# SHI-Labs/Self-Similarity-Grouping

Hardware: AMD Instinct MI355X
Metric: images/s embed + s/iter for NxN rerank+DBSCAN, N=16k, 1/2/4/8 GPU (higher is better)
Workload: dtype f32 (embed: split-half operands hi+lo on fp16 MFMA, fp32 accumulate, 6e-8 max error vs the fp32 reference features) / exact int64 via int8 MFMA digits + f64 + f16 (distance, re-rank: half semantics, bit-exact)

## Files before the change

### self-similarity-grouping_amd/csrc/bottleneck.hip

```cpp
#include "ssg_common.h"
#include <cstdlib>

#ifndef SSG_BN_NT_STORE
#define SSG_BN_NT_STORE 1
#endif
#ifndef SSG_BN_NT_RES
#define SSG_BN_NT_RES 1
#endif

namespace ssg {
namespace bneck {

typedef float v16f __attribute__((ext_vector_type(16)));
typedef unsigned int v4u __attribute__((ext_vector_type(4)));
typedef _Float16 v8h __attribute__((ext_vector_type(8)));
typedef float v4f __attribute__((ext_vector_type(4)));

struct Params {
  const float* x; float* out;
  const float* w1; const float* b1; const float* cs1;
  const float* w2; const float* b2; const float* cs2;
  const float* w3; const float* b3; const float* cs3;
  int B, H;
  int* overflow;
  unsigned long long* prof = nullptr;
};
#ifdef SSG_BN_PROF
#define SSG_BN_STAMP(I_) { if (p.prof && threadIdx.x == 0) p.prof[(size_t)blockIdx.x * 8 + (I_)] = __builtin_readcyclecounter(); }
#else
#define SSG_BN_STAMP(I_)
#endif

constexpr int cmax(int a, int b) { return a > b ? a : b; }

template <int C, int MID, int IW, int TH, int CIN = C, int NW = 4>
struct Cfg {
  static constexpr int HROWS = TH + 2, NPIX1 = HROWS * IW, NPIX = TH * IW;
  static constexpr int NTHR = NW * 64, RPP = NTHR / 4;
#ifndef SSG_BN_K1T
#define SSG_BN_K1T 32
#endif
#ifndef SSG_BN_K1T4
#define SSG_BN_K1T4 32
#endif
  static constexpr int K1T = NW == 8 ? SSG_BN_K1T : SSG_BN_K1T4, KS1 = K1T / 16, CPR1 = 4 * KS1, RPP1 = NTHR / CPR1;
  static constexpr int XROWS = (NPIX1 + RPP1 - 1) / RPP1 * RPP1;
  static constexpr int P1 = 80;
  static constexpr int P1T = K1T * 4 + 16;
  static constexpr int KT2 = NW == 8 ? 2 : 1;
  static constexpr int P2 = KT2 * 128 + 16;
  static constexpr int PY = MID * 4 + 16;
  static constexpr int BUF1 = (XROWS + MID) * P1T;
  static constexpr int ZERO_OFF = NPIX1 * PY;
  static constexpr int W2_OFF = (ZERO_OFF + PY + 255) / 256 * 256, BUF2 = MID * P2;
  static constexpr int W3_OFF = (NPIX * PY + 255) / 256 * 256, BUF3 = C * P1;
  static constexpr int LDS = cmax(cmax(2 * BUF1, W2_OFF + 2 * BUF2), W3_OFF + 2 * BUF3);
  static constexpr int DS = CIN != C;
#ifdef SSG_BN_ABL_NK1
  static constexpr int NK1 = SSG_BN_ABL_NK1;
#else
  static constexpr int NK1 = CIN / K1T;
#endif
  static constexpr int NK2 = (MID / 32) * 9 / KT2, NK3 = (MID + (DS ? CIN : 0)) / 16;
  static constexpr int PD1MAX = K1T == 64 ? 2 : (K1T == 32 ? 4 : 8);
  static constexpr int PD1 = NK1 < PD1MAX ? NK1 : PD1MAX, PD2 = KT2 == 1 ? 6 : 3;
  static_assert(((MID / 32) * 9) % KT2 == 0 && NK2 % PD2 == 0, "phase-2 stages and ring");
  static_assert((NW == 4 || NW == 8) && NPIX == 128 && NPIX1 % 32 == 0 && MID % RPP == 0 && MID % RPP1 == 0 && C % RPP == 0 && MID % (NW * 8) == 0, "128 output pixels, whole staging passes");
  static constexpr bool ZERO_EARLY = 2 * BUF1 <= ZERO_OFF;
  static_assert(LDS <= (NW == 4 ? 80 : 160) * 1024, "4 waves: two workgroups per CU; 8 waves: one");
  static_assert(NW == 4 || NW * 32 * 36 * 4 <= 2 * BUF3, "8 waves: the epilogue patches take over the W3 stages");
};

__device__ __forceinline__ unsigned pack2(_Float16 a, _Float16 b) {
  return (unsigned)__builtin_bit_cast(unsigned short, a) | ((unsigned)__builtin_bit_cast(unsigned short, b) << 16);
}
__device__ __forceinline__ void encode4(const float4 v, uint2& hi, uint2& lo) {
  const _Float16 h0 = (_Float16)v.x, h1 = (_Float16)v.y, h2 = (_Float16)v.z, h3 = (_Float16)v.w;
  hi = make_uint2(pack2(h0, h1), pack2(h2, h3));
  lo = make_uint2(pack2((_Float16)(v.x - (float)h0), (_Float16)(v.y - (float)h1)), pack2((_Float16)(v.z - (float)h2), (_Float16)(v.w - (float)h3)));
}
__device__ __forceinline__ unsigned hi_nonfinite_bits(const uint2 hi) {
  return ((hi.x & 0x7c007c00u) + 0x04000400u) | ((hi.y & 0x7c007c00u) + 0x04000400u);
}
__device__ __forceinline__ float hlo(unsigned u) { return (float)__builtin_bit_cast(_Float16, (unsigned short)(u & 0xffffu)); }
__device__ __forceinline__ float hhi(unsigned u) { return (float)__builtin_bit_cast(_Float16, (unsigned short)(u >> 16)); }
__device__ __forceinline__ float4 decode4(const uint2 hi, const uint2 lo) {
  return make_float4(hlo(hi.x) + hlo(lo.x), hhi(hi.x) + hhi(lo.x), hlo(hi.y) + hlo(lo.y), hhi(hi.y) + hhi(lo.y));
}
__device__ __forceinline__ float4 relu4(float4 v) {
  return make_float4(v.x > 0.f ? v.x : 0.f, v.y > 0.f ? v.y : 0.f, v.z > 0.f ? v.z : 0.f, v.w > 0.f ? v.w : 0.f);
}

__device__ __forceinline__ void bn_dma16(const __amdgpu_buffer_rsrc_t r, unsigned lds_addr, unsigned voff, int soff) {
  __builtin_amdgcn_raw_ptr_buffer_load_lds(r, (__attribute__((address_space(3))) void*)(uintptr_t)lds_addr, 16, voff, soff, 0, 0);
}

template <int C, int MID, int IW, int TH, int CIN, int NW>
__global__ __launch_bounds__(NW * 64, NW == 4 ? 2 : 1) void bottleneck_kernel(Params p) {
  using K = Cfg<C, MID, IW, TH, CIN, NW>;
  constexpr bool DS = K::DS;
  extern __shared__ __attribute__((aligned(16))) unsigned char smem[];
  const int tid = (int)threadIdx.x, lane = tid & 63, wave = tid >> 6, l32 = lane & 31, h = lane >> 5;
  const int tiles_img = p.H / TH, ntiles = p.B * tiles_img;
  int T;
  {
    const int b = (int)blockIdx.x, q = ntiles / 8, r = ntiles % 8, x = b % 8, s = b / 8;
    T = (x < r ? x * (q + 1) : r * (q + 1) + (x - r) * q) + s;
  }
  const int img = T / tiles_img, ty0 = (T - img * tiles_img) * TH;
  SSG_BN_STAMP(0)
  if (K::ZERO_EARLY && tid < K::PY / 16) *reinterpret_cast<uint4*>(smem + K::ZERO_OFF + tid * 16) = make_uint4(0u, 0u, 0u, 0u);

  constexpr int RPP = K::RPP, RPP1 = K::RPP1, AU = K::XROWS / RPP1, WU = MID / RPP1;
  const int ck = tid & 3, r0 = tid >> 2;
  const int ck1 = tid % K::CPR1, r1 = tid / K::CPR1;
  const float* ximg = p.x + (int64_t)img * p.H * IW * CIN;
  const __amdgpu_buffer_rsrc_t xrsrc = __builtin_amdgcn_make_buffer_rsrc(const_cast<float*>(ximg), 0, (unsigned)(p.H * IW * CIN * 4), 0x00020000);
  constexpr int MT1 = K::NPIX1 / 32, NT1 = MID / 32;
  constexpr int WC1 = NT1 < NW / 2 ? NT1 : NW / 2, WR1 = NW / WC1, MTW1 = (MT1 + WR1 - 1) / WR1, NTW1 = NT1 / WC1;
  static_assert(NT1 % WC1 == 0 && (WR1 * MTW1) * 32 <= K::XROWS, "phase-1 tiles divide over the waves");
  const int i1b = (wave / WC1) * MTW1, j1b = (wave % WC1) * NTW1;
  v16f acc1[MTW1][NTW1];
#pragma unroll
  for (int i = 0; i < MTW1; i++)
#pragma unroll
    for (int j = 0; j < NTW1; j++)
#pragma unroll
      for (int r = 0; r < 16; r++) acc1[i][j][r] = 0.f;
  float4 cs1r[NTW1][4], b1r[NTW1][4];
#pragma unroll
  for (int j = 0; j < NTW1; j++)
#pragma unroll
    for (int q = 0; q < 4; q++) {
      cs1r[j][q] = *reinterpret_cast<const float4*>(p.cs1 + (j1b + j) * 32 + 8 * q + 4 * h); b1r[j][q] = *reinterpret_cast<const float4*>(p.b1 + (j1b + j) * 32 + 8 * q + 4 * h);
    }
#ifndef SSG_BN_P1DMA
#define SSG_BN_P1DMA 1
#endif
  if constexpr (NW == 8 && K::K1T == 32 && SSG_BN_P1DMA) {
    constexpr int NS = 4, XR = K::NPIX1, SROWS = XR + MID, STG = SROWS * 128, NBLK = SROWS / 8, TDMA = (NBLK + NW - 1) / NW;
    static_assert(K::NK1 % NS == 0 && NS * STG <= K::LDS && SROWS % 8 == 0 && XR % 8 == 0 && MTW1 == 3 && NTW1 == 1, "phase-1 DMA stages");
    const int wv = __builtin_amdgcn_readfirstlane(wave);
    const __amdgpu_buffer_rsrc_t wrsrc = __builtin_amdgcn_make_buffer_rsrc(const_cast<float*>(p.w1), 0, (unsigned)(MID * CIN * 4), 0x00020000);
    unsigned go[TDMA];
    int gblk[TDMA];
#pragma unroll
    for (int u = 0; u < TDMA; u++) {
      int blk = wv + NW * u;
      if (blk >= NBLK) blk = wv;
      gblk[u] = blk;
      const int r = blk * 8 + (lane >> 3), lc = (lane & 7) ^ ((r >> 1) & 7);
      if (blk < XR / 8) {
        const int pix = (ty0 - 1) * IW + r;
        go[u] = (pix >= 0 && pix < p.H * IW) ? (unsigned)((pix * CIN + lc * 4) * 4) : 0x80000000u;
      } else {
        go[u] = (unsigned)(((r - XR) * CIN + lc * 4) * 4);
      }
    }
#define SSG_BN_DMA1(T_, ST_)                                                                                         \
    { _Pragma("unroll") for (int u = 0; u < TDMA; u++)                                                               \
        bn_dma16(gblk[u] < XR / 8 ? xrsrc : wrsrc, (unsigned)(uintptr_t)(smem + (ST_) * STG + gblk[u] * 1024), go[u], (T_) * 128); }
    const int i1s = __builtin_amdgcn_readfirstlane(i1b);
    int xo[MTW1], xs[MTW1];
#pragma unroll
    for (int i = 0; i < MTW1; i++) { const int r = (i1s + i) * 32 + l32; xo[i] = r * 128; xs[i] = (r >> 1) & 7; }
    const int wr_ = XR + j1b * 32 + l32, wo = wr_ * 128, ws = (wr_ >> 1) & 7;
    v8h fxh[2][2][MTW1], fxl[2][2][MTW1], fwh[2][2], fwl[2][2];
#define SSG_BN_READS1(ST_, S_)                                                                                       \
    { const unsigned char* sb_ = smem + (ST_) * STG;                                                                 \
      _Pragma("unroll") for (int ks = 0; ks < 2; ks++) {                                                             \
        _Pragma("unroll") for (int i = 0; i < MTW1; i++) {                                        \
          fxh[S_][ks][i] = *reinterpret_cast<const v8h*>(sb_ + xo[i] + (((4 * ks + 2 * h) ^ xs[i]) * 16));           \
          fxl[S_][ks][i] = *reinterpret_cast<const v8h*>(sb_ + xo[i] + (((4 * ks + 2 * h + 1) ^ xs[i]) * 16)); }     \
        fwh[S_][ks] = *reinterpret_cast<const v8h*>(sb_ + wo + (((4 * ks + 2 * h) ^ ws) * 16));                       \
        fwl[S_][ks] = *reinterpret_cast<const v8h*>(sb_ + wo + (((4 * ks + 2 * h + 1) ^ ws) * 16)); } }
#define SSG_BN_MMAK(S_, KS_)                                                                                         \
    { _Pragma("unroll") for (int i = 0; i < MTW1; i++) acc1[i][0] = __builtin_amdgcn_mfma_f32_32x32x16_f16(fwh[S_][KS_], fxl[S_][KS_][i], acc1[i][0], 0, 0, 0); \
      _Pragma("unroll") for (int i = 0; i < MTW1; i++) acc1[i][0] = __builtin_amdgcn_mfma_f32_32x32x16_f16(fwl[S_][KS_], fxh[S_][KS_][i], acc1[i][0], 0, 0, 0); \
      _Pragma("unroll") for (int i = 0; i < MTW1; i++) acc1[i][0] = __builtin_amdgcn_mfma_f32_32x32x16_f16(fwh[S_][KS_], fxh[S_][KS_][i], acc1[i][0], 0, 0, 0); }
#define SSG_BN_STEPD(KT_, ST_, STN_, S_)                                                                             \
    { SSG_BN_MMAK(S_, 0)                                                                                             \
      __builtin_amdgcn_sched_barrier(0);                                                                             \
      asm volatile("s_waitcnt vmcnt(%0) lgkmcnt(0)\n\ts_barrier" ::"n"(TDMA * (NS - 2)) : "memory");                  \
      { const int tn_ = (KT_) + NS < K::NK1 ? (KT_) + NS : K::NK1 - 1;    \
        SSG_BN_DMA1(tn_, ST_) }                                                                                      \
      SSG_BN_READS1(STN_, 1 - (S_))                                                                                  \
      __builtin_amdgcn_sched_barrier(0);                                                                             \
      SSG_BN_MMAK(S_, 1) }
    SSG_BN_DMA1(0, 0) SSG_BN_DMA1(1, 1) SSG_BN_DMA1(2, 2) SSG_BN_DMA1(3, 3)
    asm volatile("s_waitcnt vmcnt(%0)\n\ts_barrier" ::"n"(TDMA * (NS - 1)) : "memory");
    SSG_BN_READS1(0, 0)
#pragma unroll 1
    for (int kt = 0; kt < K::NK1; kt += NS) {
      SSG_BN_STEPD(kt, 0, 1, 0) SSG_BN_STEPD(kt + 1, 1, 2, 1) SSG_BN_STEPD(kt + 2, 2, 3, 0) SSG_BN_STEPD(kt + 3, 3, 0, 1)
    }
    __syncthreads();
#undef SSG_BN_STEPD
#undef SSG_BN_MMAK
#undef SSG_BN_READS1
#undef SSG_BN_DMA1
  } else {
  unsigned aoff[AU];
#pragma unroll
  for (int u = 0; u < AU; u++) {
    const int hp = r1 + RPP1 * u, pix = (ty0 - 1) * IW + hp;
    aoff[u] = (hp < K::NPIX1 && pix >= 0 && pix < p.H * IW) ? (unsigned)((pix * CIN + ck1 * 4) * 4) : 0x80000000u;
  }
  const float* w1p = p.w1 + (int64_t)r1 * CIN + ck1 * 4;
  v4f sa[K::PD1][AU], sw[K::PD1][WU];
#define SSG_BN_LOAD1(T_, S_)                                                                                         \
  {                                                                                                                  \
    _Pragma("unroll") for (int u = 0; u < AU; u++) {                                                                  \
      const v4u raw = __builtin_amdgcn_raw_buffer_load_b128(xrsrc, aoff[u], (T_) * (K::K1T * 4), 0);                  \
      sa[S_][u] = __builtin_bit_cast(v4f, raw);                                                                     \
    }                                                                                                                 \
    _Pragma("unroll") for (int u = 0; u < WU; u++) sw[S_][u] = *reinterpret_cast<const v4f*>(w1p + (int64_t)(RPP1 * u) * CIN + (T_) * K::K1T); \
  }
#define SSG_BN_STORE1(BUF_, S_)                                                                                      \
  {                                                                                                                  \
    unsigned char* sb_ = smem + (BUF_) * K::BUF1;                                                                    \
    _Pragma("unroll") for (int u = 0; u < AU; u++) *reinterpret_cast<v4f*>(sb_ + (r1 + RPP1 * u) * K::P1T + ck1 * 16) = sa[S_][u]; \
    _Pragma("unroll") for (int u = 0; u < WU; u++) *reinterpret_cast<v4f*>(sb_ + (K::XROWS + r1 + RPP1 * u) * K::P1T + ck1 * 16) = sw[S_][u]; \
  }
#define SSG_BN_MMA1(BUF_)                                                                                            \
  {                                                                                                                  \
    const unsigned char* sb_ = smem + (BUF_) * K::BUF1;                                                              \
    _Pragma("unroll") for (int ks = 0; ks < K::KS1; ks++) {                                                          \
    v8h xh_[MTW1], xl_[MTW1], wh_[NTW1], wl_[NTW1];                                                                  \
    _Pragma("unroll") for (int i = 0; i < MTW1; i++) {                                                               \
      const unsigned char* q_ = sb_ + ((i1b + i) * 32 + l32) * K::P1T + ks * 64 + h * 32;                            \
      xh_[i] = *reinterpret_cast<const v8h*>(q_); xl_[i] = *reinterpret_cast<const v8h*>(q_ + 16); }                 \
    _Pragma("unroll") for (int j = 0; j < NTW1; j++) {                                                               \
      const unsigned char* q_ = sb_ + (K::XROWS + (j1b + j) * 32 + l32) * K::P1T + ks * 64 + h * 32;                 \
      wh_[j] = *reinterpret_cast<const v8h*>(q_); wl_[j] = *reinterpret_cast<const v8h*>(q_ + 16); }                 \
    _Pragma("unroll") for (int i = 0; i < MTW1; i++) _Pragma("unroll") for (int j = 0; j < NTW1; j++)                \
      acc1[i][j] = __builtin_amdgcn_mfma_f32_32x32x16_f16(wh_[j], xl_[i], acc1[i][j], 0, 0, 0);                      \
    _Pragma("unroll") for (int i = 0; i < MTW1; i++) _Pragma("unroll") for (int j = 0; j < NTW1; j++)                \
      acc1[i][j] = __builtin_amdgcn_mfma_f32_32x32x16_f16(wl_[j], xh_[i], acc1[i][j], 0, 0, 0);                      \
    _Pragma("unroll") for (int i = 0; i < MTW1; i++) _Pragma("unroll") for (int j = 0; j < NTW1; j++)                \
      acc1[i][j] = __builtin_amdgcn_mfma_f32_32x32x16_f16(wh_[j], xh_[i], acc1[i][j], 0, 0, 0);                      \
    }                                                                                                                \
  }
#define SSG_BN_STEP1(KT_, S_)                                                                                        \
  {                                                                                                                  \
    if ((KT_) + K::PD1 < K::NK1) SSG_BN_LOAD1((KT_) + K::PD1, S_)    \
    SSG_BN_MMA1((S_) & 1)                                                                                            \
    if ((KT_) + 1 < K::NK1) SSG_BN_STORE1(((S_) + 1) & 1, ((S_) + 1) % K::PD1)                                        \
    __syncthreads();                                                                                                 \
  }
  static_assert(K::NK1 % K::PD1 == 0 && K::PD1 <= 8, "phase-1 ring of PD1 register sets");
#define SSG_BN_LOAD1_IF(S_) if constexpr ((S_) < K::PD1) SSG_BN_LOAD1(S_, S_)
  SSG_BN_LOAD1_IF(0) SSG_BN_LOAD1_IF(1) SSG_BN_LOAD1_IF(2) SSG_BN_LOAD1_IF(3) SSG_BN_LOAD1_IF(4) SSG_BN_LOAD1_IF(5) SSG_BN_LOAD1_IF(6) SSG_BN_LOAD1_IF(7)
#undef SSG_BN_LOAD1_IF
  SSG_BN_STORE1(0, 0)
  __syncthreads();
#define SSG_BN_STEP1_IF(KT_, S_) if constexpr ((S_) < K::PD1) SSG_BN_STEP1(KT_, S_)
#pragma unroll
  for (int kt0 = 0; kt0 < K::NK1; kt0 += K::PD1) {
    SSG_BN_STEP1_IF(kt0, 0) SSG_BN_STEP1_IF(kt0 + 1, 1) SSG_BN_STEP1_IF(kt0 + 2, 2) SSG_BN_STEP1_IF(kt0 + 3, 3)
    SSG_BN_STEP1_IF(kt0 + 4, 4) SSG_BN_STEP1_IF(kt0 + 5, 5) SSG_BN_STEP1_IF(kt0 + 6, 6) SSG_BN_STEP1_IF(kt0 + 7, 7)
  }
#undef SSG_BN_STEP1_IF
#undef SSG_BN_STEP1
  }
  SSG_BN_STAMP(1)
#undef SSG_BN_LOAD1
#undef SSG_BN_STORE1
#undef SSG_BN_MMA1

  constexpr int CPR2 = 8 * K::KT2, RP8 = K::NTHR / CPR2, BU = MID / RP8;
  const int ck8 = tid % CPR2, r8 = tid / CPR2;
  const float* w2p = p.w2 + (int64_t)r8 * (9 * MID) + ck8 * 4;
  v4f sb2[K::PD2][BU];
#define SSG_BN_LOAD2(T_, S_)                                                                                         \
  { _Pragma("unroll") for (int u = 0; u < BU; u++) sb2[S_][u] = *reinterpret_cast<const v4f*>(w2p + (int64_t)(RP8 * u) * (9 * MID) + (T_) * (32 * K::KT2)); }
#define SSG_BN_STORE2(BUF_, S_)                                                                                      \
  { unsigned char* sb_ = smem + K::W2_OFF + (BUF_) * K::BUF2;                                                        \
    _Pragma("unroll") for (int u = 0; u < BU; u++) *reinterpret_cast<v4f*>(sb_ + (r8 + RP8 * u) * K::P2 + ck8 * 16) = sb2[S_][u]; }
#define SSG_BN_LOAD2_IF(S_) if constexpr ((S_) < K::PD2) SSG_BN_LOAD2(S_, S_)
  SSG_BN_LOAD2_IF(0) SSG_BN_LOAD2_IF(1) SSG_BN_LOAD2_IF(2) SSG_BN_LOAD2_IF(3) SSG_BN_LOAD2_IF(4) SSG_BN_LOAD2_IF(5)
#undef SSG_BN_LOAD2_IF

  unsigned ovf = 0u;
#pragma unroll
  for (int i = 0; i < MTW1; i++) {
    if (i1b + i >= MT1) continue;
    const int hp0 = (i1b + i) * 32;
    const int irow = ty0 - 1 + (hp0 + l32) / IW;
    const bool inside = irow >= 0 && irow < p.H;
#pragma unroll
    for (int j = 0; j < NTW1; j++)
#pragma unroll
      for (int q = 0; q < 4; q++) {
        const int ch = (j1b + j) * 32 + 8 * q + 4 * h;
        const float4 cs = cs1r[j][q], bi = b1r[j][q];
        float4 v = make_float4(acc1[i][j][4 * q] * cs.x + bi.x, acc1[i][j][4 * q + 1] * cs.y + bi.y, acc1[i][j][4 * q + 2] * cs.z + bi.z,
                               acc1[i][j][4 * q + 3] * cs.w + bi.w);
        v = relu4(v);
        if (!inside) v = make_float4(0.f, 0.f, 0.f, 0.f);
        uint2 hi, lo;
        encode4(v, hi, lo);
        ovf |= hi_nonfinite_bits(hi);
        unsigned char* d = smem + (hp0 + l32) * K::PY + (ch >> 3) * 32 + h * 8;
        *reinterpret_cast<uint2*>(d) = hi; *reinterpret_cast<uint2*>(d + 16) = lo;
      }
  }
  if (!K::ZERO_EARLY && tid < K::PY / 16) *reinterpret_cast<uint4*>(smem + K::ZERO_OFF + tid * 16) = make_uint4(0u, 0u, 0u, 0u);
  SSG_BN_STORE2(0, 0)
  __syncthreads();
  SSG_BN_STAMP(2)

  constexpr int WC2 = NW / 4, NT2 = MID / 32 / WC2;
  const int pt2 = wave / WC2, cb2 = (wave % WC2) * NT2;
  v16f acc2[NT2];
#pragma unroll
  for (int j = 0; j < NT2; j++)
#pragma unroll
    for (int r = 0; r < 16; r++) acc2[j][r] = 0.f;
  const int m2 = pt2 * 32 + l32, ty2 = m2 / IW, tx2 = m2 - ty2 * IW;
  float4 cs2r[NT2][4], b2r[NT2][4];
#pragma unroll
  for (int j = 0; j < NT2; j++)
#pragma unroll
    for (int q = 0; q < 4; q++) {
      cs2r[j][q] = *reinterpret_cast<const float4*>(p.cs2 + (cb2 + j) * 32 + 8 * q + 4 * h); b2r[j][q] = *reinterpret_cast<const float4*>(p.b2 + (cb2 + j) * 32 + 8 * q + 4 * h);
    }
#define SSG_BN_STEP2(KT_, S_, B_)                                                                                     \
  {                                                                                                                  \
    if ((KT_) + K::PD2 < K::NK2) SSG_BN_LOAD2((KT_) + K::PD2, S_)                                                     \
    _Pragma("unroll") for (int sub = 0; sub < K::KT2; sub++) {                                                       \
      const int kt_ = (KT_) * K::KT2 + sub;                                                                          \
      const int chunk = kt_ / 9, tap = kt_ - chunk * 9, r = tap / 3, s = tap - r * 3;                                \
      const int xin = tx2 + s - 1;                                                                                   \
      const int abase = (xin >= 0 && xin < IW) ? ((ty2 + r) * IW + xin) * K::PY : K::ZERO_OFF;                       \
      const unsigned char* wb = smem + K::W2_OFF + (B_) * K::BUF2 + (cb2 * 32 + l32) * K::P2 + sub * 128 + h * 32;     \
      v8h xh_[2], xl_[2], wh_[2][NT2], wl_[2][NT2];                                                                  \
      _Pragma("unroll") for (int ks = 0; ks < 2; ks++) {                                                             \
        const unsigned char* q_ = smem + abase + (chunk * 4 + ks * 2 + h) * 32;                                      \
        xh_[ks] = *reinterpret_cast<const v8h*>(q_); xl_[ks] = *reinterpret_cast<const v8h*>(q_ + 16);               \
        _Pragma("unroll") for (int j = 0; j < NT2; j++) {                                                            \
          wh_[ks][j] = *reinterpret_cast<const v8h*>(wb + j * 32 * K::P2 + ks * 64);                                 \
          wl_[ks][j] = *reinterpret_cast<const v8h*>(wb + j * 32 * K::P2 + ks * 64 + 16); }                          \
      }                                                                                                              \
      _Pragma("unroll") for (int ks = 0; ks < 2; ks++) {                                                             \
        _Pragma("unroll") for (int j = 0; j < NT2; j++) acc2[j] = __builtin_amdgcn_mfma_f32_32x32x16_f16(wh_[ks][j], xl_[ks], acc2[j], 0, 0, 0); \
        _Pragma("unroll") for (int j = 0; j < NT2; j++) acc2[j] = __builtin_amdgcn_mfma_f32_32x32x16_f16(wl_[ks][j], xh_[ks], acc2[j], 0, 0, 0); \
        _Pragma("unroll") for (int j = 0; j < NT2; j++) acc2[j] = __builtin_amdgcn_mfma_f32_32x32x16_f16(wh_[ks][j], xh_[ks], acc2[j], 0, 0, 0); \
      }                                                                                                              \
    }                                                                                                                \
    if ((KT_) + 1 < K::NK2) SSG_BN_STORE2((B_) ^ 1, ((S_) + 1) % K::PD2)                                              \
    __syncthreads();                                                                                                 \
  }
  static_assert(K::NK2 % 6 == 0 && 6 % K::PD2 == 0, "phase-2 ring");
#pragma unroll
  for (int kt0 = 0; kt0 < K::NK2; kt0 += 6) {
    SSG_BN_STEP2(kt0, 0 % K::PD2, 0) SSG_BN_STEP2(kt0 + 1, 1 % K::PD2, 1) SSG_BN_STEP2(kt0 + 2, 2 % K::PD2, 0)
    SSG_BN_STEP2(kt0 + 3, 3 % K::PD2, 1) SSG_BN_STEP2(kt0 + 4, 4 % K::PD2, 0) SSG_BN_STEP2(kt0 + 5, 5 % K::PD2, 1)
  }
#undef SSG_BN_STEP2
  SSG_BN_STAMP(3)
#undef SSG_BN_LOAD2
#undef SSG_BN_STORE2

  constexpr int CU3 = C / RPP;
  constexpr int K3 = MID + (DS ? CIN : 0);
  const float* w3p = p.w3 + (int64_t)r0 * K3 + ck * 4;
  v4f sc3[2][CU3];
#define SSG_BN_LOAD3(T_, S_)                                                                                         \
  { _Pragma("unroll") for (int u = 0; u < CU3; u++) sc3[S_][u] = *reinterpret_cast<const v4f*>(w3p + (int64_t)(RPP * u) * K3 + (T_) * 16); }
#define SSG_BN_STORE3(BUF_, S_)                                                                                      \
  { unsigned char* sb_ = smem + K::W3_OFF + (BUF_) * K::BUF3;                                                        \
    _Pragma("unroll") for (int u = 0; u < CU3; u++) *reinterpret_cast<v4f*>(sb_ + (r0 + RPP * u) * K::P1 + ck * 16) = sc3[S_][u]; }
  SSG_BN_LOAD3(0, 0)
  SSG_BN_LOAD3(1, 1)
  constexpr int WC3 = NW / 4, NT3 = C / 32 / WC3;
  const int pt3 = wave / WC3, cb3 = (wave % WC3) * NT3;
  const int64_t gpix0 = ((int64_t)img * p.H + ty0) * IW + pt3 * 32;
  constexpr int NXK = DS ? CIN / 16 : 1;
  v8h xrh[NXK], xrl[NXK];
  if constexpr (DS) {
    const float* xq = p.x + (gpix0 + l32) * CIN + h * 8;
#pragma unroll
    for (int t = 0; t < NXK; t++) { xrh[t] = *reinterpret_cast<const v8h*>(xq + t * 16); xrl[t] = *reinterpret_cast<const v8h*>(xq + t * 16 + 4); }
  }
  unsigned char* myrows = smem + (pt3 * 32) * K::PY;
#pragma unroll
  for (int j = 0; j < NT2; j++)
#pragma unroll
    for (int q = 0; q < 4; q++) {
      const int ch = (cb2 + j) * 32 + 8 * q + 4 * h;
      const float4 cs = cs2r[j][q], bi = b2r[j][q];
      float4 v = make_float4(acc2[j][4 * q] * cs.x + bi.x, acc2[j][4 * q + 1] * cs.y + bi.y, acc2[j][4 * q + 2] * cs.z + bi.z, acc2[j][4 * q + 3] * cs.w + bi.w);
      v = relu4(v);
      uint2 hi, lo;
      encode4(v, hi, lo);
      ovf |= hi_nonfinite_bits(hi);
      unsigned char* d = smem + (pt2 * 32 + l32) * K::PY + (ch >> 3) * 32 + h * 8;
      *reinterpret_cast<uint2*>(d) = hi; *reinterpret_cast<uint2*>(d + 16) = lo;
    }

  static_assert(K::NK3 % 2 == 0, "phase 3 takes its k-tiles in rounds of two buffers");
  v16f acc3[NT3];
#pragma unroll
  for (int j = 0; j < NT3; j++)
#pragma unroll
    for (int r = 0; r < 16; r++) acc3[j][r] = 0.f;
#define SSG_BN_MMA3K(BUF_, KT_)                                                                                      \
  {                                                                                                                  \
    v8h xh_, xl_;                                                                                                    \
    if constexpr (DS && (KT_) >= MID / 16) { xh_ = xrh[((KT_) - MID / 16) % NXK]; xl_ = xrl[((KT_) - MID / 16) % NXK]; } \
    else {                                                                                                           \
      const unsigned char* q_ = myrows + l32 * K::PY + (((KT_) % (MID / 16)) * 2 + h) * 32;                          \
      xh_ = *reinterpret_cast<const v8h*>(q_); xl_ = *reinterpret_cast<const v8h*>(q_ + 16);                         \
    }                                                                                                                \
    const unsigned char* wb_ = smem + K::W3_OFF + (BUF_) * K::BUF3 + (cb3 * 32 + l32) * K::P1 + h * 32;              \
    _Pragma("unroll") for (int jj = 0; jj < NT3; jj += 4) {                                                          \
      v8h wh_[4], wl_[4];                                                                                            \
      _Pragma("unroll") for (int j = 0; j < 4; j++) {                                                                \
        wh_[j] = *reinterpret_cast<const v8h*>(wb_ + (jj + j) * 32 * K::P1); wl_[j] = *reinterpret_cast<const v8h*>(wb_ + (jj + j) * 32 * K::P1 + 16); } \
      _Pragma("unroll") for (int j = 0; j < 4; j++) acc3[jj + j] = __builtin_amdgcn_mfma_f32_32x32x16_f16(wh_[j], xl_, acc3[jj + j], 0, 0, 0); \
      _Pragma("unroll") for (int j = 0; j < 4; j++) acc3[jj + j] = __builtin_amdgcn_mfma_f32_32x32x16_f16(wl_[j], xh_, acc3[jj + j], 0, 0, 0); \
      _Pragma("unroll") for (int j = 0; j < 4; j++) acc3[jj + j] = __builtin_amdgcn_mfma_f32_32x32x16_f16(wh_[j], xh_, acc3[jj + j], 0, 0, 0); \
    }                                                                                                                \
  }
  constexpr int EP = 36, CPR = 8, RPI = 8, ITS = 4;
  const int chunk = lane % CPR, prow = lane / CPR, odd = lane & 1;
  const float* __restrict__ resp = p.x + gpix0 * C;
  float* __restrict__ outp = p.out + gpix0 * C;
  float4 rr[2][ITS], b3r[2], cs3r[2];
#ifdef SSG_BN_ABL_NORES
#define SSG_BN_RESLOAD(P_) make_float4(0.f, 0.f, 0.f, 0.f)
#elif SSG_BN_NT_RES
#define SSG_BN_RESLOAD(P_) ([&]() { const v4f t_ = __builtin_nontemporal_load(reinterpret_cast<const v4f*>(P_)); return make_float4(t_[0], t_[1], t_[2], t_[3]); }())
#else
#define SSG_BN_RESLOAD(P_) (*reinterpret_cast<const float4*>(P_))
#endif
  SSG_BN_STORE3(0, 0)
  SSG_BN_STORE3(1, 1)
  if constexpr (K::NK3 > 2) { SSG_BN_LOAD3(2, 0) SSG_BN_LOAD3(3, 1) }
  __syncthreads();
  static_assert(K::NK3 / 2 <= 4, "at most four rounds");
#define SSG_BN_ROUND3(R_)                                                                                            \
  if constexpr ((R_) < K::NK3 / 2) {                                                                                 \
    SSG_BN_MMA3K(0, 2 * (R_))                                                                                        \
    SSG_BN_MMA3K(1, 2 * (R_) + 1)                                                                                    \
    if constexpr ((R_) + 1 < K::NK3 / 2) {                                                                           \
      __syncthreads();                                                \
      SSG_BN_STORE3(0, 0)                                                                                            \
      SSG_BN_STORE3(1, 1)                                                                                            \
      if constexpr ((R_) + 2 < K::NK3 / 2) { SSG_BN_LOAD3(2 * (R_) + 4, 0) SSG_BN_LOAD3(2 * (R_) + 5, 1) }           \
      else {                                  \
        if constexpr (!DS) {                                                                                         \
          _Pragma("unroll") for (int it = 0; it < ITS; it++) rr[0][it] = SSG_BN_RESLOAD(resp + (int64_t)(it * RPI + prow) * C + cb3 * 32 + chunk * 4); \
        }                                                                                                            \
        b3r[0] = *reinterpret_cast<const float4*>(p.b3 + cb3 * 32 + chunk * 4); cs3r[0] = *reinterpret_cast<const float4*>(p.cs3 + cb3 * 32 + chunk * 4); \
      }                                                                                                              \
      __syncthreads();                                                                                               \
    }                                                                                                                \
  }
  SSG_BN_ROUND3(0) SSG_BN_ROUND3(1) SSG_BN_ROUND3(2) SSG_BN_ROUND3(3)
#undef SSG_BN_ROUND3
  SSG_BN_STAMP(4)
#undef SSG_BN_LOAD3
#undef SSG_BN_STORE3
#undef SSG_BN_MMA3K

  static_assert(32 * EP * 4 <= 32 * K::PY, "patch fits in the wave's y2 rows");
  float* patch;
  if constexpr (WC3 == 1) patch = reinterpret_cast<float*>(myrows);
  else {
    __syncthreads();
    patch = reinterpret_cast<float*>(smem + K::W3_OFF) + wave * (32 * EP);
  }
#pragma unroll
  for (int j = 0; j < NT3; j++) {
    const int col = (cb3 + j) * 32 + chunk * 4;
    if (j + 1 < NT3) {
      if constexpr (!DS) {
#pragma unroll
        for (int it = 0; it < ITS; it++) rr[(j + 1) & 1][it] = SSG_BN_RESLOAD(resp + (int64_t)(it * RPI + prow) * C + col + 32);
      }
      b3r[(j + 1) & 1] = *reinterpret_cast<const float4*>(p.b3 + col + 32); cs3r[(j + 1) & 1] = *reinterpret_cast<const float4*>(p.cs3 + col + 32);
    }
    const float4 bias = b3r[j & 1], cs = cs3r[j & 1];
#pragma unroll
    for (int q = 0; q < 4; q++)
      *reinterpret_cast<float4*>(patch + l32 * EP + 8 * q + 4 * h) = make_float4(acc3[j][4 * q], acc3[j][4 * q + 1], acc3[j][4 * q + 2], acc3[j][4 * q + 3]);
    __builtin_amdgcn_fence(__ATOMIC_ACQ_REL, "wavefront");
#pragma unroll
    for (int it = 0; it < ITS; it++) {
      const int pr = it * RPI + prow;
      float4 v = *reinterpret_cast<const float4*>(patch + pr * EP + chunk * 4);
      v.x = v.x * cs.x + bias.x; v.y = v.y * cs.y + bias.y; v.z = v.z * cs.z + bias.z; v.w = v.w * cs.w + bias.w;
      if constexpr (!DS) {
      const float4 rw = rr[j & 1][it];
      float4 r4;
      {
        const unsigned a0 = __float_as_uint(rw.x), a1 = __float_as_uint(rw.y), a2 = __float_as_uint(rw.z), a3 = __float_as_uint(rw.w);
        const unsigned g0 = lane_xor1((odd ? a0 : a2)), g1 = lane_xor1((odd ? a1 : a3));
        const unsigned h0 = odd ? g0 : a0, h1 = odd ? g1 : a1, l0 = odd ? a2 : g0, l1 = odd ? a3 : g1;
        r4 = decode4(make_uint2(h0, h1), make_uint2(l0, l1));
      }
      v.x += r4.x; v.y += r4.y; v.z += r4.z; v.w += r4.w;
      }
      v = relu4(v);
      uint2 hp, lp;
      encode4(v, hp, lp);
      ovf |= hi_nonfinite_bits(hp);
      const unsigned rx = lane_xor1((odd ? hp.x : lp.x)), ry = lane_xor1((odd ? hp.y : lp.y));
      const uint4 stv = make_uint4(odd ? rx : hp.x, odd ? ry : hp.y, odd ? lp.x : rx, odd ? lp.y : ry);
#if SSG_BN_NT_STORE
      { const v4u sv_ = {stv.x, stv.y, stv.z, stv.w}; __builtin_nontemporal_store(sv_, reinterpret_cast<v4u*>(outp + (int64_t)pr * C + col)); }
#else
      *reinterpret_cast<uint4*>(outp + (int64_t)pr * C + col) = stv;
#endif
    }
    __builtin_amdgcn_fence(__ATOMIC_ACQ_REL, "wavefront");
  }
  if ((ovf & 0x80008000u) && p.overflow) *p.overflow = 1;
  SSG_BN_STAMP(5)
}

}
}

extern "C" int ssg_bottleneck_supported(int H, int W, int CIN, int C, int MID) {
  if (C == 256 && MID == 64 && (CIN == 256 || CIN == 64) && W == 32 && H > 0 && H % 4 == 0) return 1;
  if (C == 512 && MID == 128 && CIN == 512 && W == 16 && H > 0 && H % 8 == 0) return 1;
  return 0;
}

template <int C, int MID, int IW, int TH, int CIN, int NW>
static int launch_bottleneck(const ssg::bneck::Params& p, hipStream_t stream) {
  using namespace ssg::bneck;
  using K = Cfg<C, MID, IW, TH, CIN, NW>;
  static bool attr_set = false;
  if (!attr_set) {
    SSG_HIP(hipFuncSetAttribute((const void*)bottleneck_kernel<C, MID, IW, TH, CIN, NW>, hipFuncAttributeMaxDynamicSharedMemorySize, K::LDS));
    attr_set = true;
  }
  hipLaunchKernelGGL((bottleneck_kernel<C, MID, IW, TH, CIN, NW>), dim3(p.B * (p.H / TH)), dim3(NW * 64), K::LDS, stream, p);
  SSG_LAUNCH_CHECK("bottleneck_kernel");
  return SSG_OK;
}

extern "C" int ssg_bottleneck_nhwc_x(const void* x, const void* w1, const float* b1, const float* cs1, const void* w2, const float* b2, const float* cs2,
                                     const void* w3, const float* b3, const float* cs3, void* out, int B, int H, int W, int C, int MID,
                                     int32_t* overflow, hipStream_t stream) {
  using namespace ssg::bneck;
  if (B <= 0 || !ssg_bottleneck_supported(H, W, C, C, MID) || !cs1 || !cs2 || !cs3 || x == out) {
    ssg_set_error("ssg_bottleneck_nhwc_x: unsupported block B=%d H=%d W=%d C=%d MID=%d (see ssg_bottleneck_supported)", B, H, W, C, MID);
    return SSG_ERR_INVALID;
  }
  Params p;
  p.x = (const float*)x; p.out = (float*)out;
  p.w1 = (const float*)w1; p.b1 = b1; p.cs1 = cs1; p.w2 = (const float*)w2; p.b2 = b2; p.cs2 = cs2; p.w3 = (const float*)w3; p.b3 = b3; p.cs3 = cs3;
  p.B = B; p.H = H; p.overflow = overflow;
  if (C == 512) return launch_bottleneck<512, 128, 16, 8, 512, 8>(p, stream);
  return launch_bottleneck<256, 64, 32, 4, 256, 4>(p, stream);
}

extern "C" int ssg_bottleneck_ds_nhwc_x(const void* x, const void* w1, const float* b1, const float* cs1, const void* w2, const float* b2, const float* cs2,
                                        const void* w3cat, const float* b3, const float* cs3, void* out, int B, int H, int W, int CIN, int C, int MID,
                                        int32_t* overflow, hipStream_t stream) {
  using namespace ssg::bneck;
  if (B <= 0 || CIN == C || !ssg_bottleneck_supported(H, W, CIN, C, MID) || !cs1 || !cs2 || !cs3) {
    ssg_set_error("ssg_bottleneck_ds_nhwc_x: unsupported block B=%d H=%d W=%d CIN=%d C=%d MID=%d (see ssg_bottleneck_supported)", B, H, W, CIN, C, MID);
    return SSG_ERR_INVALID;
  }
  Params p;
  p.x = (const float*)x; p.out = (float*)out;
  p.w1 = (const float*)w1; p.b1 = b1; p.cs1 = cs1; p.w2 = (const float*)w2; p.b2 = b2; p.cs2 = cs2; p.w3 = (const float*)w3cat; p.b3 = b3; p.cs3 = cs3;
  p.B = B; p.H = H; p.overflow = overflow;
  return launch_bottleneck<256, 64, 32, 4, 64, 4>(p, stream);
}
```

Measured before the change: 27570.

## Split bottleneck phase-3 into channel groups and overlap epilogue with next group's MMAs

Phase 3 (the 1x1 expand conv plus residual epilogue) now runs over output-channel groups, four by default. The epilogue of one group (scale, bias, residual decode, relu, split-half encode, nontemporal store) is interleaved with the MFMA stages of the next group, and the residual loads are prefetched several tiles ahead. The goal is to hide the serial epilogue and its global memory traffic behind matrix work, and to shrink the W3 staging buffers so a dedicated per-wave patch area fits in LDS. In exchange the stage count rises and so do register pressure and the number of syncs, and the macro logic is intricate.

```diff
diff --git a/self-similarity-grouping_amd/csrc/bottleneck.hip b/self-similarity-grouping_amd/csrc/bottleneck.hip
--- a/self-similarity-grouping_amd/csrc/bottleneck.hip
+++ b/self-similarity-grouping_amd/csrc/bottleneck.hip
@@ -6,6 +6,12 @@
 #endif
 #ifndef SSG_BN_NT_RES
 #define SSG_BN_NT_RES 1
+#endif
+#ifndef SSG_BN_P3_GROUPS
+#define SSG_BN_P3_GROUPS 4
+#endif
+#ifndef SSG_BN_RES_AHEAD
+#define SSG_BN_RES_AHEAD 3
 #endif
 
 namespace ssg {
@@ -54,7 +60,9 @@
   static constexpr int ZERO_OFF = NPIX1 * PY;
   static constexpr int W2_OFF = (ZERO_OFF + PY + 255) / 256 * 256, BUF2 = MID * P2;
   static constexpr int W3_OFF = (NPIX * PY + 255) / 256 * 256, BUF3 = C * P1;
-  static constexpr int LDS = cmax(cmax(2 * BUF1, W2_OFF + 2 * BUF2), W3_OFF + 2 * BUF3);
+  static constexpr int G3 = SSG_BN_P3_GROUPS, KPS3 = G3 >= 4 ? G3 / 2 : 1, BUF3G = KPS3 * (C / G3) * P1, PATCH_OFF = W3_OFF + 2 * BUF3G, PATCH = 32 * 36 * 4;
+  static constexpr int P3_END = G3 > 1 ? PATCH_OFF + NW * PATCH : W3_OFF + 2 * BUF3;
+  static constexpr int LDS = cmax(cmax(2 * BUF1, W2_OFF + 2 * BUF2), P3_END);
   static constexpr int DS = CIN != C;
 #ifdef SSG_BN_ABL_NK1
   static constexpr int NK1 = SSG_BN_ABL_NK1;
@@ -68,7 +76,8 @@
   static_assert((NW == 4 || NW == 8) && NPIX == 128 && NPIX1 % 32 == 0 && MID % RPP == 0 && MID % RPP1 == 0 && C % RPP == 0 && MID % (NW * 8) == 0, "128 output pixels, whole staging passes");
   static constexpr bool ZERO_EARLY = 2 * BUF1 <= ZERO_OFF;
   static_assert(LDS <= (NW == 4 ? 80 : 160) * 1024, "4 waves: two workgroups per CU; 8 waves: one");
-  static_assert(NW == 4 || NW * 32 * 36 * 4 <= 2 * BUF3, "8 waves: the epilogue patches take over the W3 stages");
+  static_assert(G3 > 1 || NW == 4 || NW * 32 * 36 * 4 <= 2 * BUF3, "8 waves, one group: the epilogue patches take over the W3 stages");
+  static_assert((G3 == 1 || G3 == 2 || G3 == 4) && NK3 % KPS3 == 0 && (C / 32 / (NW / 4)) % G3 == 0 && (C / G3) % RPP == 0 && RPP % 32 == 0, "phase-3 channel groups: whole channel tiles, whole staging passes");
 };
 
 __device__ __forceinline__ unsigned pack2(_Float16 a, _Float16 b) {
@@ -93,6 +102,33 @@
 
 __device__ __forceinline__ void bn_dma16(const __amdgpu_buffer_rsrc_t r, unsigned lds_addr, unsigned voff, int soff) {
   __builtin_amdgcn_raw_ptr_buffer_load_lds(r, (__attribute__((address_space(3))) void*)(uintptr_t)lds_addr, 16, voff, soff, 0, 0);
+}
+
+template <bool RES>
+__device__ __forceinline__ void epi_row(float4 v, const float4 cs, const float4 bias, const float4 rw, const int odd,
+                                        float* __restrict__ dst, unsigned& ovf) {
+  v.x = v.x * cs.x + bias.x; v.y = v.y * cs.y + bias.y; v.z = v.z * cs.z + bias.z; v.w = v.w * cs.w + bias.w;
+  if constexpr (RES) {
+    float4 r4;
+    {
+      const unsigned a0 = __float_as_uint(rw.x), a1 = __float_as_uint(rw.y), a2 = __float_as_uint(rw.z), a3 = __float_as_uint(rw.w);
+      const unsigned g0 = lane_xor1((odd ? a0 : a2)), g1 = lane_xor1((odd ? a1 : a3));
+      const unsigned h0 = odd ? g0 : a0, h1 = odd ? g1 : a1, l0 = odd ? a2 : g0, l1 = odd ? a3 : g1;
+      r4 = decode4(make_uint2(h0, h1), make_uint2(l0, l1));
+    }
+    v.x += r4.x; v.y += r4.y; v.z += r4.z; v.w += r4.w;
+  }
+  v = relu4(v);
+  uint2 hp, lp;
+  encode4(v, hp, lp);
+  ovf |= hi_nonfinite_bits(hp);
+  const unsigned rx = lane_xor1((odd ? hp.x : lp.x)), ry = lane_xor1((odd ? hp.y : lp.y));
+  const uint4 stv = make_uint4(odd ? rx : hp.x, odd ? ry : hp.y, odd ? lp.x : rx, odd ? lp.y : ry);
+#if SSG_BN_NT_STORE
+  { const v4u sv_ = {stv.x, stv.y, stv.z, stv.w}; __builtin_nontemporal_store(sv_, reinterpret_cast<v4u*>(dst)); }
+#else
+  *reinterpret_cast<uint4*>(dst) = stv;
+#endif
 }
 
 template <int C, int MID, int IW, int TH, int CIN, int NW>
@@ -362,6 +398,7 @@
 #undef SSG_BN_LOAD2
 #undef SSG_BN_STORE2
 
+#if SSG_BN_P3_GROUPS == 1
   constexpr int CU3 = C / RPP;
   constexpr int K3 = MID + (DS ? CIN : 0);
   const float* w3p = p.w3 + (int64_t)r0 * K3 + ck * 4;
@@ -373,6 +410,24 @@
     _Pragma("unroll") for (int u = 0; u < CU3; u++) *reinterpret_cast<v4f*>(sb_ + (r0 + RPP * u) * K::P1 + ck * 16) = sc3[S_][u]; }
   SSG_BN_LOAD3(0, 0)
   SSG_BN_LOAD3(1, 1)
+#else
+  constexpr int G3 = K::G3, KPS = K::KPS3, SPG = K::NK3 / KPS, CU3 = C / G3 / RPP;
+  constexpr int K3 = MID + (DS ? CIN : 0);
+  constexpr int NTG = C / 32 / (NW / 4) / G3, NU3 = G3 * SPG, PD3 = 4;
+  static_assert(NU3 <= 16 && NU3 >= PD3 && NTG <= SPG && KPS <= 2, "phase-3 stages");
+  const float* w3p[CU3];
+#pragma unroll
+  for (int u = 0; u < CU3; u++) { const int r = r0 + RPP * u; w3p[u] = p.w3 + (int64_t)((r / (32 * NTG)) * (G3 * 32 * NTG) + r % (32 * NTG)) * K3 + ck * 4; }
+  v4f sc3[PD3][KPS][CU3];
+#define SSG_BN_LOAD3(Q_, S_)                                                                                         \
+  { _Pragma("unroll") for (int k = 0; k < KPS; k++) _Pragma("unroll") for (int u = 0; u < CU3; u++)                   \
+      sc3[S_][k][u] = *reinterpret_cast<const v4f*>(w3p[u] + ((Q_) / SPG) * (32 * NTG * K3) + (((Q_) % SPG) * KPS + k) * 16); }
+#define SSG_BN_STORE3(BUF_, S_)                                                                                      \
+  { unsigned char* sb_ = smem + K::W3_OFF + (BUF_) * K::BUF3G;                                                       \
+    _Pragma("unroll") for (int k = 0; k < KPS; k++) _Pragma("unroll") for (int u = 0; u < CU3; u++)                   \
+      *reinterpret_cast<v4f*>(sb_ + (k * (C / G3) + r0 + RPP * u) * K::P1 + ck * 16) = sc3[S_][k][u]; }
+  SSG_BN_LOAD3(0, 0) SSG_BN_LOAD3(1, 1) SSG_BN_LOAD3(2, 2) SSG_BN_LOAD3(3, 3)
+#endif
   constexpr int WC3 = NW / 4, NT3 = C / 32 / WC3;
   const int pt3 = wave / WC3, cb3 = (wave % WC3) * NT3;
   const int64_t gpix0 = ((int64_t)img * p.H + ty0) * IW + pt3 * 32;
@@ -399,6 +454,18 @@
       *reinterpret_cast<uint2*>(d) = hi; *reinterpret_cast<uint2*>(d + 16) = lo;
     }
 
+  constexpr int EP = 36, CPR = 8, RPI = 8, ITS = 4;
+  const int chunk = lane % CPR, prow = lane / CPR, odd = lane & 1;
+  const float* __restrict__ resp = p.x + gpix0 * C;
+  float* __restrict__ outp = p.out + gpix0 * C;
+#ifdef SSG_BN_ABL_NORES
+#define SSG_BN_RESLOAD(P_) make_float4(0.f, 0.f, 0.f, 0.f)
+#elif SSG_BN_NT_RES
+#define SSG_BN_RESLOAD(P_) ([&]() { const v4f t_ = __builtin_nontemporal_load(reinterpret_cast<const v4f*>(P_)); return make_float4(t_[0], t_[1], t_[2], t_[3]); }())
+#else
+#define SSG_BN_RESLOAD(P_) (*reinterpret_cast<const float4*>(P_))
+#endif
+#if SSG_BN_P3_GROUPS == 1
   static_assert(K::NK3 % 2 == 0, "phase 3 takes its k-tiles in rounds of two buffers");
   v16f acc3[NT3];
 #pragma unroll
@@ -423,18 +490,7 @@
       _Pragma("unroll") for (int j = 0; j < 4; j++) acc3[jj + j] = __builtin_amdgcn_mfma_f32_32x32x16_f16(wh_[j], xh_, acc3[jj + j], 0, 0, 0); \
     }                                                                                                                \
   }
-  constexpr int EP = 36, CPR = 8, RPI = 8, ITS = 4;
-  const int chunk = lane % CPR, prow = lane / CPR, odd = lane & 1;
-  const float* __restrict__ resp = p.x + gpix0 * C;
-  float* __restrict__ outp = p.out + gpix0 * C;
   float4 rr[2][ITS], b3r[2], cs3r[2];
-#ifdef SSG_BN_ABL_NORES
-#define SSG_BN_RESLOAD(P_) make_float4(0.f, 0.f, 0.f, 0.f)
-#elif SSG_BN_NT_RES
-#define SSG_BN_RESLOAD(P_) ([&]() { const v4f t_ = __builtin_nontemporal_load(reinterpret_cast<const v4f*>(P_)); return make_float4(t_[0], t_[1], t_[2], t_[3]); }())
-#else
-#define SSG_BN_RESLOAD(P_) (*reinterpret_cast<const float4*>(P_))
-#endif
   SSG_BN_STORE3(0, 0)
   SSG_BN_STORE3(1, 1)
   if constexpr (K::NK3 > 2) { SSG_BN_LOAD3(2, 0) SSG_BN_LOAD3(3, 1) }
@@ -461,6 +517,7 @@
   SSG_BN_ROUND3(0) SSG_BN_ROUND3(1) SSG_BN_ROUND3(2) SSG_BN_ROUND3(3)
 #undef SSG_BN_ROUND3
   SSG_BN_STAMP(4)
+  SSG_BN_STAMP(5)
 #undef SSG_BN_LOAD3
 #undef SSG_BN_STORE3
 #undef SSG_BN_MMA3K
@@ -490,35 +547,109 @@
 #pragma unroll
     for (int it = 0; it < ITS; it++) {
       const int pr = it * RPI + prow;
-      float4 v = *reinterpret_cast<const float4*>(patch + pr * EP + chunk * 4);
-      v.x = v.x * cs.x + bias.x; v.y = v.y * cs.y + bias.y; v.z = v.z * cs.z + bias.z; v.w = v.w * cs.w + bias.w;
-      if constexpr (!DS) {
-      const float4 rw = rr[j & 1][it];
-      float4 r4;
-      {
-        const unsigned a0 = __float_as_uint(rw.x), a1 = __float_as_uint(rw.y), a2 = __float_as_uint(rw.z), a3 = __float_as_uint(rw.w);
-        const unsigned g0 = lane_xor1((odd ? a0 : a2)), g1 = lane_xor1((odd ? a1 : a3));
-        const unsigned h0 = odd ? g0 : a0, h1 = odd ? g1 : a1, l0 = odd ? a2 : g0, l1 = odd ? a3 : g1;
-        r4 = decode4(make_uint2(h0, h1), make_uint2(l0, l1));
-      }
-      v.x += r4.x; v.y += r4.y; v.z += r4.z; v.w += r4.w;
-      }
-      v = relu4(v);
-      uint2 hp, lp;
-      encode4(v, hp, lp);
-      ovf |= hi_nonfinite_bits(hp);
-      const unsigned rx = lane_xor1((odd ? hp.x : lp.x)), ry = lane_xor1((odd ? hp.y : lp.y));
-      const uint4 stv = make_uint4(odd ? rx : hp.x, odd ? ry : hp.y, odd ? lp.x : rx, odd ? lp.y : ry);
-#if SSG_BN_NT_STORE
-      { const v4u sv_ = {stv.x, stv.y, stv.z, stv.w}; __builtin_nontemporal_store(sv_, reinterpret_cast<v4u*>(outp + (int64_t)pr * C + col)); }
-#else
-      *reinterpret_cast<uint4*>(outp + (int64_t)pr * C + col) = stv;
-#endif
+      epi_row<!DS>(*reinterpret_cast<const float4*>(patch + pr * EP + chunk * 4), cs, bias, rr[j & 1][it], odd, outp + (int64_t)pr * C + col, ovf);
     }
     __builtin_amdgcn_fence(__ATOMIC_ACQ_REL, "wavefront");
   }
+#else
+  constexpr int HS3 = 2 * NTG, NE3 = 2 * NT3, RD3 = SSG_BN_RES_AHEAD < NE3 ? SSG_BN_RES_AHEAD : NE3, RS3 = RD3 + 1;
+  static_assert(RD3 >= 1 && RD3 <= 8, "residual prefetch distance");
+  v16f acc3[2][NTG];
+  float4 rr[RS3][2], b3r[2], cs3r[2], pv[2];
+  float* const patch = reinterpret_cast<float*>(smem + K::PATCH_OFF) + wave * (32 * EP);
+#define SSG_BN_MMA3K(BUF_, Q_, KK_)                                                                                  \
+  {                                                                                                                  \
+    constexpr int kt_ = ((Q_) % SPG) * KPS + (KK_), a_ = ((Q_) / SPG) & 1;                                           \
+    if constexpr (kt_ == 0) {                                                                                        \
+      _Pragma("unroll") for (int j = 0; j < NTG; j++) _Pragma("unroll") for (int r = 0; r < 16; r++) acc3[a_][j][r] = 0.f; }  \
+    v8h xh_, xl_, wh_[NTG], wl_[NTG];                                                                                \
+    if constexpr (DS && kt_ >= MID / 16) { xh_ = xrh[(kt_ - MID / 16) % NXK]; xl_ = xrl[(kt_ - MID / 16) % NXK]; }   \
+    else {                                                                                                           \
+      const unsigned char* q_ = myrows + l32 * K::PY + ((kt_ % (MID / 16)) * 2 + h) * 32;                            \
+      xh_ = *reinterpret_cast<const v8h*>(q_); xl_ = *reinterpret_cast<const v8h*>(q_ + 16);                         \
+    }                                                                                                                \
+    const unsigned char* wb_ = smem + K::W3_OFF + (BUF_) * K::BUF3G + ((KK_) * (C / G3) + (wave % WC3) * NTG * 32 + l32) * K::P1 + h * 32; \
+    _Pragma("unroll") for (int j = 0; j < NTG; j++) {                                                                \
+      wh_[j] = *reinterpret_cast<const v8h*>(wb_ + j * 32 * K::P1); wl_[j] = *reinterpret_cast<const v8h*>(wb_ + j * 32 * K::P1 + 16); } \
+    _Pragma("unroll") for (int j = 0; j < NTG; j++) acc3[a_][j] = __builtin_amdgcn_mfma_f32_32x32x16_f16(wh_[j], xl_, acc3[a_][j], 0, 0, 0); \
+    _Pragma("unroll") for (int j = 0; j < NTG; j++) acc3[a_][j] = __builtin_amdgcn_mfma_f32_32x32x16_f16(wl_[j], xh_, acc3[a_][j], 0, 0, 0); \
+    _Pragma("unroll") for (int j = 0; j < NTG; j++) acc3[a_][j] = __builtin_amdgcn_mfma_f32_32x32x16_f16(wh_[j], xh_, acc3[a_][j], 0, 0, 0); \
+  }
+#define SSG_BN_RES3(E_)                                                                                              \
+  { _Pragma("unroll") for (int i2 = 0; i2 < 2; i2++)                                                                 \
+      rr[(E_) % RS3][i2] = SSG_BN_RESLOAD(resp + (int64_t)((((E_) & 1) * 2 + i2) * RPI + prow) * C + (cb3 + (E_) / 2) * 32 + chunk * 4); }
+#define SSG_BN_EPI3_A(E_)                                                                                            \
+  {                                                                                                                  \
+    constexpr int jt_ = (E_) / 2, a_ = ((E_) / HS3) & 1, j_ = jt_ % NTG, hf_ = (E_) & 1;                             \
+    if constexpr (!DS && (E_) + RD3 < NE3) SSG_BN_RES3((E_) + RD3)                                                   \
+    if constexpr (hf_ == 0) {                                                                                        \
+      if constexpr (jt_ + 1 < NT3) {                                                                                 \
+        b3r[(jt_ + 1) & 1] = *reinterpret_cast<const float4*>(p.b3 + (cb3 + jt_ + 1) * 32 + chunk * 4);              \
+        cs3r[(jt_ + 1) & 1] = *reinterpret_cast<const float4*>(p.cs3 + (cb3 + jt_ + 1) * 32 + chunk * 4); }          \
+      _Pragma("unroll") for (int q = 0; q < 4; q++)                                                                  \
+        *reinterpret_cast<float4*>(patch + l32 * EP + 8 * q + 4 * h) = make_float4(acc3[a_][j_][4 * q], acc3[a_][j_][4 * q + 1], acc3[a_][j_][4 * q + 2], acc3[a_][j_][4 * q + 3]); \
+      __builtin_amdgcn_fence(__ATOMIC_ACQ_REL, "wavefront");                                                         \
+    }                                                                                                                \
+    _Pragma("unroll") for (int i2 = 0; i2 < 2; i2++) pv[i2] = *reinterpret_cast<const float4*>(patch + ((hf_ * 2 + i2) * RPI + prow) * EP + chunk * 4); \
+  }
+#define SSG_BN_EPI3_R(E_, I2_)                                                                                       \
+  {                                                                                                                  \
+    constexpr int jt_ = (E_) / 2;                                                                                    \
+    const int pr = (((E_) & 1) * 2 + (I2_)) * RPI + prow;                                                            \
+    epi_row<!DS>(pv[I2_], cs3r[jt_ & 1], b3r[jt_ & 1], rr[(E_) % RS3][I2_], odd, outp + (int64_t)pr * C + (cb3 + jt_) * 32 + chunk * 4, ovf); \
+  }
+#define SSG_BN_EPI3_Z(E_) { if constexpr (((E_) & 1) == 1) __builtin_amdgcn_fence(__ATOMIC_ACQ_REL, "wavefront"); }
+#define SSG_BN_EPI3(E_) { SSG_BN_EPI3_A(E_) SSG_BN_EPI3_R(E_, 0) SSG_BN_EPI3_R(E_, 1) SSG_BN_EPI3_Z(E_) }
+#define SSG_BN_EPI3_AT(PC_, Q_, I_)                                                                                  \
+  if constexpr ((Q_) >= SPG && ((Q_) % SPG) * HS3 / SPG + (I_) < ((Q_) % SPG + 1) * HS3 / SPG)                       \
+    PC_(((Q_) / SPG - 1) * HS3 + ((Q_) % SPG) * HS3 / SPG + (I_))
+#define SSG_BN_EPI3_R0(E_) SSG_BN_EPI3_R(E_, 0)
+#define SSG_BN_EPI3_R1(E_) SSG_BN_EPI3_R(E_, 1)
+#define SSG_BN_RES3_IF(E_) if constexpr (!DS && (E_) < RD3) SSG_BN_RES3(E_)
+#define SSG_BN_STAGE3(Q_)                                                                                            \
+  if constexpr ((Q_) < NU3) {                                                                                        \
+    if constexpr ((Q_) + PD3 < NU3) SSG_BN_LOAD3((Q_) + PD3, (Q_) % PD3)    \
+    if constexpr ((Q_) == (SPG > 1 ? SPG - 2 : 0)) {                                      \
+      SSG_BN_RES3_IF(0) SSG_BN_RES3_IF(1) SSG_BN_RES3_IF(2) SSG_BN_RES3_IF(3) SSG_BN_RES3_IF(4) SSG_BN_RES3_IF(5) SSG_BN_RES3_IF(6) SSG_BN_RES3_IF(7) \
+      b3r[0] = *reinterpret_cast<const float4*>(p.b3 + cb3 * 32 + chunk * 4); cs3r[0] = *reinterpret_cast<const float4*>(p.cs3 + cb3 * 32 + chunk * 4); \
+    }                                                                                                                \
+    SSG_BN_EPI3_AT(SSG_BN_EPI3_A, Q_, 0)                                                                             \
+    SSG_BN_MMA3K((Q_) & 1, Q_, 0)                                                                                    \
+    SSG_BN_EPI3_AT(SSG_BN_EPI3_R0, Q_, 0)                                                                            \
+    if constexpr (KPS > 1) SSG_BN_MMA3K((Q_) & 1, Q_, 1)                                                             \
+    SSG_BN_EPI3_AT(SSG_BN_EPI3_R1, Q_, 0) SSG_BN_EPI3_AT(SSG_BN_EPI3_Z, Q_, 0)                                       \
+    SSG_BN_EPI3_AT(SSG_BN_EPI3, Q_, 1)                                                                               \
+    if constexpr ((Q_) + 1 < NU3) {                                                                                  \
+      SSG_BN_STORE3(((Q_) + 1) & 1, ((Q_) + 1) % PD3)                                                                \
+      __syncthreads();                                                                                               \
+    }                                                                                                                \
+    if constexpr ((Q_) == SPG - 1) { SSG_BN_STAMP(4) }                                     \
+  }
+#define SSG_BN_STAGE3X4(Q_) SSG_BN_STAGE3(Q_) SSG_BN_STAGE3((Q_) + 1) SSG_BN_STAGE3((Q_) + 2) SSG_BN_STAGE3((Q_) + 3)
+  SSG_BN_STORE3(0, 0)
+  __syncthreads();
+  SSG_BN_STAGE3X4(0) SSG_BN_STAGE3X4(4) SSG_BN_STAGE3X4(8) SSG_BN_STAGE3X4(12)
+  SSG_BN_STAMP(5)
+#define SSG_BN_EPI3_TAIL(L_) if constexpr ((L_) < HS3) SSG_BN_EPI3((G3 - 1) * HS3 + (L_))
+  SSG_BN_EPI3_TAIL(0) SSG_BN_EPI3_TAIL(1) SSG_BN_EPI3_TAIL(2) SSG_BN_EPI3_TAIL(3) SSG_BN_EPI3_TAIL(4) SSG_BN_EPI3_TAIL(5) SSG_BN_EPI3_TAIL(6) SSG_BN_EPI3_TAIL(7)
+#undef SSG_BN_EPI3_TAIL
+#undef SSG_BN_STAGE3X4
+#undef SSG_BN_STAGE3
+#undef SSG_BN_RES3_IF
+#undef SSG_BN_EPI3_AT
+#undef SSG_BN_EPI3
+#undef SSG_BN_EPI3_A
+#undef SSG_BN_EPI3_R
+#undef SSG_BN_EPI3_R0
+#undef SSG_BN_EPI3_R1
+#undef SSG_BN_EPI3_Z
+#undef SSG_BN_RES3
+#undef SSG_BN_MMA3K
+#undef SSG_BN_LOAD3
+#undef SSG_BN_STORE3
+#endif
   if ((ovf & 0x80008000u) && p.overflow) *p.overflow = 1;
-  SSG_BN_STAMP(5)
+  SSG_BN_STAMP(6)
 }
 
 }
```

After: 27810, median of 6. About the same (+0.8%).
